# sunchao/leveldb-rs

Hardware: AMD Instinct MI355X
Metric: GiB/s device-resident batched CRC32C, 4KiB blocks; %HBM-peak at 1/2/4/8 GPUs (higher is better)
Workload: dtype u32

## Files before the change

leveldb-rs_amd/csrc/lvk/knobs.h:

```cpp
#pragma once

#if !defined(LVK_EXPERIMENT_BUILD) && ( \
    defined(LVK_STAGGER) || \
    defined(LVK_AL_ROWS) || \
    defined(LVK_MAX_PIECES) || \
    defined(LVK_WAL_TOUCH_HOPS) || \
    defined(LVK_SMALL_WAVES) || \
    defined(LVK_SEAL_FLUSH) || \
    defined(LVK_SST_ROWS) || \
    defined(LVK_SEAL_ROWS) || \
    defined(LVK_SST_RUN) || \
    defined(LVK_SORT_MIN_WGS) || \
    defined(LVK_SMALL_ROUNDS) || \
    defined(LVK_HASH_WGS_PER_CU) || \
    defined(LVK_PIPE_CHUNK_MB) || \
    defined(LVK_PIPE_FIRST_MB) || \
    defined(LVK_MEMCPY_THREADS) || \
    defined(LVK_PIPE_COPY_THREADS) || \
    defined(LVK_WAL_UNSORT) || \
    defined(LVK_MT_TILE) || \
    defined(LVK_MT_PREFIX) || \
    defined(LVK_SB_TILE) || \
    defined(LVK_SB_WAVE_COPY) || \
    defined(LVK_SB_COPY_LANES))
#error "LVK_* kernel switches select untested code paths; only experiment variants (LVK_EXPERIMENT_BUILD, tools/build_variant.sh) may set them"
#endif

#ifndef LVK_STAGGER
#define LVK_STAGGER 1u
#endif
#ifndef LVK_AL_ROWS
#define LVK_AL_ROWS 4
#endif
#ifndef LVK_MAX_PIECES
#define LVK_MAX_PIECES 4096
#endif
#ifndef LVK_WAL_TOUCH_HOPS
#define LVK_WAL_TOUCH_HOPS 16
#endif
#ifndef LVK_SMALL_WAVES
#define LVK_SMALL_WAVES 4
#endif
#ifndef LVK_SEAL_FLUSH
#define LVK_SEAL_FLUSH 16
#endif
#ifndef LVK_SST_ROWS
#define LVK_SST_ROWS 3
#endif
#ifndef LVK_SEAL_ROWS
#define LVK_SEAL_ROWS LVK_SST_ROWS
#endif
#ifndef LVK_SST_RUN
#define LVK_SST_RUN 4
#endif
#ifndef LVK_SORT_MIN_WGS
#define LVK_SORT_MIN_WGS 1024
#endif
#ifndef LVK_SMALL_ROUNDS
#define LVK_SMALL_ROUNDS 52
#endif
#ifndef LVK_PIPE_CHUNK_MB
#define LVK_PIPE_CHUNK_MB 32
#endif
#ifndef LVK_PIPE_FIRST_MB
#define LVK_PIPE_FIRST_MB 2
#endif
#ifndef LVK_MEMCPY_THREADS
#define LVK_MEMCPY_THREADS 8
#endif
#ifndef LVK_PIPE_COPY_THREADS
#define LVK_PIPE_COPY_THREADS 4
#endif
#ifndef LVK_HASH_WGS_PER_CU
#define LVK_HASH_WGS_PER_CU 8
#endif
#ifndef LVK_WAL_UNSORT
#define LVK_WAL_UNSORT 1
#endif
#ifndef LVK_MT_TILE
#define LVK_MT_TILE 512
#endif
#ifndef LVK_MT_PREFIX
#define LVK_MT_PREFIX 16
#endif
#ifndef LVK_SB_TILE
#define LVK_SB_TILE 1024
#endif
#ifndef LVK_SB_WAVE_COPY
#define LVK_SB_WAVE_COPY 64
#endif
#ifndef LVK_SB_COPY_LANES
#define LVK_SB_COPY_LANES 16
#endif
```

leveldb-rs_amd/csrc/wal_decode.hip:

```cpp
#include <hip/hip_runtime.h>

#include <algorithm>
#include <string>

#include "../../include/lvgpu/crc32c.h"
#include "../../include/lvgpu/wal.h"
#include "lv_internal.h"
#include "lvh.h"
#include "lvk/sort.h"

namespace lvk {

constexpr uint32_t kDecThreads = 256;
constexpr uint32_t kDecPer = 4;
constexpr uint32_t kDecTile = kDecThreads * kDecPer;
constexpr uint32_t kDecBlock = 32768;
constexpr uint32_t kDecHeader = 7;
constexpr uint32_t kDecMaxFrags = kDecBlock / kDecHeader + 1;
constexpr uint64_t kDecNone = ~0ull;

enum : uint32_t {
    kEvSkip = 0,
    kEvFull = 1,
    kEvFirst = 2,
    kEvMiddle = 3,
    kEvLast = 4,
    kEvType0 = 5,
    kEvUnknown = 6,
    kEvBadZero = 7,
    kEvBadLen = 8,
    kEvBadCrc = 9,
    kEvEof = 10,
    kEvStop = 11,
};

constexpr uint32_t kOpConst = 1, kOpIn = 2, kOpStop = 4;
struct DecOp {
    uint32_t flags;
    uint32_t pad;
    uint64_t size;
    uint64_t start;
};

__device__ __forceinline__ DecOp dec_ident() { return DecOp{0u, 0u, 0ull, 0ull}; }
__device__ __forceinline__ DecOp dec_closed() { return DecOp{kOpConst, 0u, 0ull, 0ull}; }

__device__ __forceinline__ DecOp dec_compose(const DecOp &a, const DecOp &b) {
    if (a.flags & kOpStop) return a;
    if (b.flags & kOpConst) return b;
    DecOp r = a;
    if (!(a.flags & kOpConst) || (a.flags & kOpIn)) r.size += b.size;
    return r;
}

__device__ __forceinline__ DecOp dec_event_op(uint32_t code, uint32_t x, uint64_t hdr) {
    if (code == kEvSkip) return dec_ident();
    if (code == kEvMiddle) return DecOp{0u, 0u, x, 0ull};
    if (code == kEvFirst) return DecOp{kOpConst | kOpIn, 0u, x, hdr};
    if (code == kEvStop) return DecOp{kOpConst | kOpStop, 0u, 0ull, 0ull};
    return dec_closed();
}

// ... 428 lines not shown
        for (uint32_t j = 0; j < kDecPer; ++j) {
            before[j] = (s.flags & kOpIn) ? s.size : kDecNone;
            if (s.flags & kOpStop) code[j] = kEvSkip;
            dec_step(code[j], x[j], hdr[j], &s, &v[j]);
            dec_accumulate(&sum, v[j]);
        }
        DecSum stotal;
        const DecSum ex = dec_scan_sum(sum, s_sum, &stotal);
        uint32_t all;
        uint32_t next = dec_next_nonzero(cfirst, s_code, &all);
        if (!next) next = ti.next_code;
        uint32_t nx[kDecPer];
#pragma unroll
        for (int j = kDecPer - 1; j >= 0; --j) {
            nx[j] = next;
            if (code[j] != kEvSkip && code[j] != kEvMiddle) next = code[j];
        }
        uint64_t R = ti.recs + ex.recs, P = ti.pay + ex.pay, Q = ti.reps + ex.reps;
#pragma unroll
        for (uint32_t j = 0; j < kDecPer; ++j) {
            const uint64_t i = tile * kDecTile + t * kDecPer + j;
            if (i >= n) break;
            for (uint32_t r = 0; r < v[j].nrep; ++r, ++Q) {
                if (!A.out.d_rep_bytes || Q >= A.out.rep_cap) continue;
                A.out.d_rep_bytes[Q] = v[j].rb[r];
                A.out.d_rep_reason[Q] = v[j].rr[r];
                A.out.d_rep_log_off[Q] = hdr[j];
            }
            uint64_t fp = kDecNone;
            if (code[j] == kEvFull)
                fp = P;
            else if (code[j] == kEvFirst && nx[j] == kEvLast)
                fp = P;
            else if (code[j] == kEvMiddle && before[j] != kDecNone && nx[j] == kEvLast)
                fp = P + before[j];
            else if (code[j] == kEvLast && before[j] != kDecNone)
                fp = P + before[j];
            A.fpos[i] = fp;
            if (v[j].emit) {
                if (R < A.out.rec_cap) {
                    A.out.d_rec_off[R] = P;
                    A.out.d_rec_len[R] = v[j].emit_len;
                    A.out.d_rec_log_off[R] = v[j].rec_log;
                }
                ++R;
                P += v[j].emit_len;
            }
        }
    }
}

typedef uint32_t dec_u4 __attribute__((ext_vector_type(4)));

__global__ __launch_bounds__(kDecThreads) void wal_unframe_kernel(const DecArgs A) {
    __shared__ uint16_t s_out[kDecMaxFrags + 1];
    __shared__ uint16_t s_src[kDecMaxFrags];
    __shared__ uint32_t s_wt[kDecThreads / 64];
    __shared__ uint64_t s_span;
    if (A.head->status) return;
    const uint32_t tid = threadIdx.x;
    const uint64_t n = A.head->n;
    const uint64_t nblocks = A.nblocks < A.nb ? A.nblocks : A.nb;
    for (uint64_t blk = blockIdx.x; blk < nblocks; blk += gridDim.x) {
        const uint32_t e0 = A.bfirst[blk], e1 = A.bend[blk];
        uint32_t cnt = 0;
        if (e0 != ~0u && e1 != ~0u && e1 > e0 && e1 <= n) cnt = e1 - e0 < kDecMaxFrags ? e1 - e0 : kDecMaxFrags;
        const uint64_t start = blk * kDecBlock;
        __syncthreads();
        uint32_t carry = 0;
        for (uint32_t k0 = 0; k0 < cnt; k0 += kDecThreads) {
            const uint32_t k = k0 + tid;
            uint32_t ll = 0;
            uint64_t fp = kDecNone;
            if (k < cnt) {
                const uint64_t i = static_cast<uint64_t>(e0) + k;
                fp = A.fpos[i];
                if (fp != kDecNone) ll = (A.ev[i] >> 8) & 0xffffu;
                s_src[k] = static_cast<uint16_t>(A.hdr_off[i] - start + kDecHeader);
            }
            const uint32_t inc = wg_incl_scan<kDecThreads / 64>(ll, s_wt);
            const uint32_t o = carry + inc - ll;
            if (k < cnt) {
                s_out[k] = static_cast<uint16_t>(o);
                if (fp != kDecNone && o == 0) s_span = fp;
            }
            uint32_t tot = 0;
#pragma unroll
            for (uint32_t w = 0; w < kDecThreads / 64; ++w) tot += s_wt[w];
            carry += tot;
            __syncthreads();
        }
        if (tid == 0) s_out[cnt] = static_cast<uint16_t>(carry);
        __syncthreads();
        const uint32_t total = carry;
        if (total == 0) continue;
        const uint64_t span = s_span;
        if (span > A.out.payload_cap || total > A.out.payload_cap - span) continue;
        uint8_t *const dst = A.out.d_payload + span;
        const uint8_t *const src = A.log + start;
        const uint32_t mis = static_cast<uint32_t>(reinterpret_cast<uintptr_t>(dst) & 15u);
        uint32_t head = (16u - mis) & 15u;
        if (head > total) head = total;
        const uint32_t ngran = (head ? 1u : 0u) + (total - head + 15u) / 16u;
        for (uint32_t g = tid; g < ngran; g += kDecThreads) {
            uint32_t lo, hi;
            if (head && g == 0) {
                lo = 0;
                hi = head;
            } else {
                lo = head + (g - (head ? 1u : 0u)) * 16u;
                hi = lo + 16u < total ? lo + 16u : total;
            }
            uint32_t a = 0, b = cnt;
            while (a < b) {
                const uint32_t m = (a + b) >> 1;
                if (s_out[m] <= lo)
                    a = m + 1;
                else
                    b = m;
            }
            uint32_t f = a - 1;
            if (hi - lo == 16u && lo + 16u <= s_out[f + 1]) {
                dec_u4 v;
                __builtin_memcpy(&v, src + s_src[f] + (lo - s_out[f]), 16);
                *reinterpret_cast<dec_u4 *>(dst + lo) = v;
                continue;
            }
            uint64_t wlo = 0, whi = 0;
            for (uint32_t p = lo; p < hi; ++p) {
                while (s_out[f + 1] <= p) ++f;
                const uint64_t byte = src[s_src[f] + (p - s_out[f])];
                const uint32_t q = p - lo;
                if (q < 8)
                    wlo |= byte << (8 * q);
                else
                    whi |= byte << (8 * (q - 8));
            }
            if (hi - lo == 16u) {
                dec_u4 v;
                v.x = static_cast<uint32_t>(wlo);
                v.y = static_cast<uint32_t>(wlo >> 32);
                v.z = static_cast<uint32_t>(whi);
                v.w = static_cast<uint32_t>(whi >> 32);
                *reinterpret_cast<dec_u4 *>(dst + lo) = v;
            } else {
                for (uint32_t q = 0; q < hi - lo; ++q)
                    dst[lo + q] = static_cast<uint8_t>((q < 8 ? wlo >> (8 * q) : whi >> (8 * (q - 8))) & 0xffu);
            }
        }
    }
}

}

using namespace lvh;

namespace {

constexpr uint64_t kMaxScanCap = 0xfffffffeull;

struct DecWs {
    size_t head, ev, fpos, blk, tsum, tin, total;
    uint64_t nb, tiles;
};
DecWs dec_ws_layout(uint64_t cap) {
    DecWs w;
    w.nb = cap + 1;
    w.tiles = (cap + lvk::kDecTile - 1) / lvk::kDecTile;
    w.head = 0;
    w.ev = al16(sizeof(lvk::DecHead));
    w.fpos = w.ev + al16(cap * sizeof(uint32_t));
    w.blk = w.fpos + al16(cap * sizeof(uint64_t));
    w.tsum = w.blk + al16(3 * w.nb * sizeof(uint32_t));
    w.tin = w.tsum + al16(w.tiles * sizeof(lvk::DecTileSum));
    w.total = w.tin + al16(w.tiles * sizeof(lvk::DecTileIn));
    return w;
}

}

extern "C" {

size_t lv_wal_decode_workspace_bytes(size_t scan_cap) { return dec_ws_layout(scan_cap).total; }

int lv_wal_decode_device(const uint8_t *d_log, size_t bytes, const uint64_t *d_hdr_off, const uint32_t *d_crc,
                         const uint32_t *d_info, const uint64_t *d_count, size_t scan_cap,
                         const lv_wal_decode_out *out, uint32_t flags, void *d_workspace, size_t workspace_bytes,
                         void *stream) {
    g_err.clear();
    if (flags & ~static_cast<uint32_t>(LV_WAL_DECODE_NO_CHECKSUM)) return set_err(LV_ERR_INVALID, "unknown flag bits");
    const bool checksum = !(flags & LV_WAL_DECODE_NO_CHECKSUM);
    if (!out) return set_err(LV_ERR_INVALID, "null output descriptor");
    if (!out->d_totals) return set_err(LV_ERR_INVALID, "null d_totals");
    if (reinterpret_cast<uintptr_t>(out->d_totals) % 8) return set_err(LV_ERR_INVALID, "d_totals must be 8-byte aligned");
    if (!d_count) return set_err(LV_ERR_INVALID, "null count pointer");
    if (!d_log && bytes) return set_err(LV_ERR_INVALID, "null log pointer");
    if (scan_cap && (!d_hdr_off || !d_info)) return set_err(LV_ERR_INVALID, "null scan array");
    if (scan_cap && checksum && !d_crc) return set_err(LV_ERR_INVALID, "null d_crc (only LV_WAL_DECODE_NO_CHECKSUM allows it)");
    if (out->payload_cap && !out->d_payload) return set_err(LV_ERR_INVALID, "null d_payload");
    if (out->rec_cap && (!out->d_rec_off || !out->d_rec_len || !out->d_rec_log_off))
// ... 65 lines not shown
```

leveldb-rs_amd/csrc/wal_encode.hip:

```cpp
#include <hip/hip_runtime.h>

#include <algorithm>
#include <cstring>
#include <mutex>
#include <vector>

#include "../../include/lvgpu/crc32c.h"
#include "../../include/lvgpu/wal.h"
#include "lv_internal.h"
#include "lvh.h"

namespace lvk {

constexpr uint32_t kFrameThreads = 256;
constexpr uint32_t kFrameBlock = 32768;
constexpr uint32_t kFrameHeader = 7;
constexpr uint32_t kFrameMaxFrags = kFrameBlock / kFrameHeader + 1;
constexpr uint64_t kFramePosMask = (1ull << 56) - 1;

struct FrameArgs {
    const uint8_t *payload;
    uint8_t *out;
    uint64_t out_len;
    uint32_t first;
    uint32_t align;
    uint64_t nblocks;
    uint64_t nfrags;
    const uint64_t *src;
    const uint64_t *pos;
    const uint32_t *len;
    const uint32_t *crc;
    const uint32_t *bidx;
};

typedef uint32_t frame_u4 __attribute__((ext_vector_type(4)));

struct FrameFrag {
    uint64_t pos, src, next;
    uint32_t len, crc, type;
};

__device__ __forceinline__ void frame_load(const FrameArgs &A, int64_t f, FrameFrag *r) {
    const uint64_t pw = A.pos[f];
    r->pos = pw & kFramePosMask;
    r->type = static_cast<uint32_t>(pw >> 56);
    r->src = A.src[f];
    r->len = A.len[f];
    r->crc = A.crc[f];
    r->next = static_cast<uint64_t>(f + 1) < A.nfrags ? (A.pos[f + 1] & kFramePosMask) : ~0ull;
}

__device__ __forceinline__ void frame_compose(const FrameArgs &A, int64_t p0, int64_t f) {
    FrameFrag r{};
    if (f >= 0)
        frame_load(A, f, &r);
    else
        r.next = A.nfrags ? (A.pos[0] & kFramePosMask) : ~0ull;
    uint64_t lo = 0, hi = 0;
    uint32_t valid = 0;
    for (uint32_t k = 0; k < 16; ++k) {
        const int64_t p = p0 + k;
        if (p < 0 || static_cast<uint64_t>(p) >= A.out_len) continue;
        valid |= 1u << k;
        while (static_cast<uint64_t>(p) >= r.next) frame_load(A, ++f, &r);
        uint32_t b = 0;
        if (f >= 0) {
            const uint64_t d = static_cast<uint64_t>(p) - r.pos;
            if (d < 4)
                b = (r.crc >> (8 * d)) & 0xffu;
            else if (d < 6)
                b = (r.len >> (8 * (d - 4))) & 0xffu;
            else if (d == 6)
                b = r.type;
            else if (d < kFrameHeader + r.len)
                b = A.payload[r.src + d - kFrameHeader];
        }
        if (k < 8)
            lo |= static_cast<uint64_t>(b) << (8 * k);
        else
            hi |= static_cast<uint64_t>(b) << (8 * (k - 8));
    }
    uint8_t *q = A.out + p0;
    if (valid == 0xffffu) {
        frame_u4 v;
        v.x = static_cast<uint32_t>(lo);
        v.y = static_cast<uint32_t>(lo >> 32);
        v.z = static_cast<uint32_t>(hi);
        v.w = static_cast<uint32_t>(hi >> 32);
        *reinterpret_cast<frame_u4 *>(q) = v;
    } else {
        for (uint32_t k = 0; k < 16; ++k)
            if (valid & (1u << k)) q[k] = static_cast<uint8_t>((k < 8 ? lo >> (8 * k) : hi >> (8 * (k - 8))) & 0xffu);
    }
}

__global__ __launch_bounds__(kFrameThreads) void wal_frame_kernel(const FrameArgs A) {
    __shared__ uint16_t s_pos[kFrameMaxFrags];
    const uint32_t tid = threadIdx.x;
    for (uint64_t blk = blockIdx.x; blk < A.nblocks; blk += gridDim.x) {
        const uint64_t lo = blk == 0 ? 0 : blk * kFrameBlock - A.first;
        const uint64_t end = (blk + 1) * kFrameBlock - A.first;
        const uint64_t hi = end < A.out_len ? end : A.out_len;
        const uint32_t f0 = A.bidx[blk];
        const uint32_t cnt = A.bidx[blk + 1] - f0;
        const uint32_t nf = cnt < kFrameMaxFrags ? cnt : kFrameMaxFrags;
        __syncthreads();
        for (uint32_t i = tid; i < nf; i += kFrameThreads)
            s_pos[i] = static_cast<uint16_t>((A.pos[f0 + i] & kFramePosMask) - lo);
        __syncthreads();
        const uint64_t g_lo = blk == 0 ? 0 : (lo + A.align + 15) / 16;
        const uint64_t g_hi = (hi + A.align + 15) / 16;
        for (uint64_t g = g_lo + tid; g < g_hi; g += kFrameThreads) {
            const int64_t p0 = static_cast<int64_t>(g * 16) - static_cast<int64_t>(A.align);
            const uint32_t rel = static_cast<uint32_t>((p0 < 0 ? 0 : p0) - static_cast<int64_t>(lo));
            uint32_t a = 0, b = nf;
            while (a < b) {
                const uint32_t m = (a + b) >> 1;
                if (s_pos[m] <= rel)
                    a = m + 1;
                else
                    b = m;
            }
            const int64_t f = static_cast<int64_t>(f0) + a - 1;
            if (a > 0 && p0 >= 0) {
                const uint32_t d = rel - s_pos[a - 1];
                const uint32_t len = A.len[f];
                if (d >= kFrameHeader && d + 16 <= kFrameHeader + len) {
                    frame_u4 v;
                    __builtin_memcpy(&v, A.payload + A.src[f] + (d - kFrameHeader), 16);
                    *reinterpret_cast<frame_u4 *>(A.out + p0) = v;
                    continue;
                }
            }
            frame_compose(A, p0, a > 0 ? f : static_cast<int64_t>(f0) - 1);
        }
    }
}

}

using namespace lvh;

namespace {

constexpr uint64_t kMaxFragments = 0xffffffffull;

struct EncWs {
    size_t src, pos, len, seed, bidx, crc, image, sort, total;
};
EncWs enc_ws_layout(uint64_t fragments) {
    EncWs w;
    w.src = 0;
    w.pos = w.src + al16(fragments * sizeof(uint64_t));
    w.len = w.pos + al16(fragments * sizeof(uint64_t));
    w.seed = w.len + al16(fragments * sizeof(uint32_t));
    w.bidx = w.seed + al16(fragments * sizeof(uint32_t));
    w.crc = w.bidx + al16((fragments + 2) * sizeof(uint32_t));
    w.image = w.crc + al16(fragments * sizeof(uint32_t));
    w.sort = w.image;
    w.total = w.sort + al16(lv_crc32c_workspace_bytes(fragments));
    return w;
}

struct StageSlot {
    uint8_t *p = nullptr;
    size_t cap = 0;
    int dev = -1;
    hipEvent_t done = nullptr;
    bool used = false;
    bool retired = false;
};
std::mutex g_stage_m;
std::vector<StageSlot> *g_stage = nullptr;

int stage_acquire(int dev, size_t need, size_t *slot) {
    if (!g_stage) g_stage = new std::vector<StageSlot>();
    std::vector<StageSlot> &v = *g_stage;
    for (size_t i = 0; i < v.size(); ++i) {
        if (v[i].dev != dev || v[i].cap < need || v[i].retired) continue;
        if (v[i].used && hipEventQuery(v[i].done) != hipSuccess) {
            (void)hipGetLastError();
            continue;
        }
        *slot = i;
        return LV_OK;
    }
    StageSlot s;
// ... 116 lines not shown
```

leveldb-rs_amd/csrc/sst_build.hip:

```cpp
#include <hip/hip_runtime.h>

#include <string>

#include "../../include/lvgpu/crc32c.h"
#include "../../include/lvgpu/table.h"
#include "lv_internal.h"
#include "lvh.h"
#include "lvk/knobs.h"

namespace lvk {

constexpr uint32_t kSbTile = LVK_SB_TILE;
constexpr uint32_t kSbWaveCopy = LVK_SB_WAVE_COPY;
constexpr uint32_t kSbCopyLanes = LVK_SB_COPY_LANES;
constexpr uint32_t kSbThreads = 256;
constexpr uint32_t kSbPer = kSbTile / kSbThreads;
constexpr uint32_t kSbMaxR = LV_SST_MAX_RESTART_INTERVAL;
constexpr uint64_t kSbLarge = 0xffffffffull;
static_assert(kSbTile % kSbThreads == 0 && kSbTile >= kSbMaxR, "a tile holds every residue of a restart interval");
static_assert(kSbTile * 16 <= 65536, "two u64 scan arrays fit the LDS a workgroup may declare");
static_assert(kSbWaveCopy >= 16, "a wave copy has at least one granule");
static_assert(kSbCopyLanes >= 16 && 64 % kSbCopyLanes == 0, "a copy's lanes cover a ragged head or tail of 15 bytes");

typedef uint32_t sb_u4 __attribute__((ext_vector_type(4)));
// ... 71 lines not shown
}

__device__ __forceinline__ void sb_put_fixed32(uint8_t *p, uint32_t v) {
    p[0] = static_cast<uint8_t>(v);
    p[1] = static_cast<uint8_t>(v >> 8);
    p[2] = static_cast<uint8_t>(v >> 16);
    p[3] = static_cast<uint8_t>(v >> 24);
}

__device__ __forceinline__ uint32_t sb_ikey_at(const uint8_t *k, uint64_t ulen, uint64_t tag, uint64_t i) {
    return i < ulen ? k[i] : static_cast<uint32_t>(tag >> (8 * (i - ulen))) & 0xffu;
}

__device__ __forceinline__ uint64_t sb_common(const uint8_t *a, const uint8_t *b, uint64_t m) {
    uint64_t i = 0;
    for (; i + 8 <= m; i += 8) {
        uint64_t x, y;
        __builtin_memcpy(&x, a + i, 8);
        __builtin_memcpy(&y, b + i, 8);
        if (x != y) return i + (static_cast<uint32_t>(__builtin_ctzll(x ^ y)) >> 3);
    }
    for (; i < m && a[i] == b[i]; ++i) {
    }
    return i;
}

__device__ __forceinline__ uint64_t sb_shared(const SbArgs &A, const lv_wb_op &p, const lv_wb_op &c) {
    const uint8_t *kp = A.payload + p.key_off, *kc = A.payload + c.key_off;
    const uint64_t m = p.key_len < c.key_len ? p.key_len : c.key_len;
    uint64_t s = sb_common(kp, kc, m);
    if (s < m) return s;
    for (uint32_t k = 0; k < 8; ++k, ++s)
        if (sb_ikey_at(kp, p.key_len, p.tag, s) != sb_ikey_at(kc, c.key_len, c.tag, s)) break;
    return s;
}

__device__ __forceinline__ void sb_tile_scan(uint64_t *s, uint32_t st, uint32_t tid) {
    for (uint32_t off = st; off < kSbTile; off <<= 1) {
        uint64_t v[kSbPer];
#pragma unroll
        for (uint32_t k = 0; k < kSbPer; ++k) {
            const uint32_t j = tid + k * kSbThreads;
            v[k] = j >= off ? s[j - off] : 0;
        }
        __syncthreads();
#pragma unroll
        for (uint32_t k = 0; k < kSbPer; ++k) s[tid + k * kSbThreads] += v[k];
        __syncthreads();
    }
}

__device__ __forceinline__ uint64_t sb_P(const SbArgs &A, uint64_t i) { return A.Pl[i] + A.cP[i / kSbTile]; }
__device__ __forceinline__ uint64_t sb_S(const SbArgs &A, uint64_t i) {
    return A.Sl[i] + A.cS[(i / kSbTile) * A.R + i % A.R];
}
__device__ __forceinline__ uint64_t sb_buffer(const SbArgs &A, uint64_t s, uint64_t e, uint64_t *restarts) {
    const uint64_t k = (e - s) / A.R, last = s + k * A.R;
    *restarts = k + 1;
    return sb_P(A, e) - (s ? sb_P(A, s - 1) : 0) + sb_S(A, last) - (s >= A.R ? sb_S(A, s - A.R) : 0);
}
__device__ __forceinline__ uint64_t sb_estimate(const SbArgs &A, uint64_t s, uint64_t e) {
    uint64_t r;
    const uint64_t b = sb_buffer(A, s, e, &r);
    return b + 4 * r + 4;
}

__global__ void sb_init(const SbArgs A) {
    SbHead h{};
    *A.head = h;
}

__global__ __launch_bounds__(kSbThreads) void sb_sizes(const SbArgs A) {
    __shared__ uint64_t s_p[kSbTile], s_s[kSbTile];
    const uint32_t tid = threadIdx.x;
    const uint64_t n = sb_entries(A);
    const uint64_t base = static_cast<uint64_t>(blockIdx.x) * kSbTile;
    if (base >= n) return;
    const uint32_t cnt = static_cast<uint32_t>(n - base < kSbTile ? n - base : kSbTile);
    int bad = 0;
#pragma unroll
    for (uint32_t k = 0; k < kSbPer; ++k) {
        const uint32_t j = tid + k * kSbThreads;
        uint64_t nr = 0, d = 0;
        if (j < cnt) {
            const uint64_t i = base + j;
            const uint32_t oi = A.order[i], pi = i ? A.order[i - 1] : oi;
            uint64_t sh = 0;
            if (oi >= A.op_cap || pi >= A.op_cap) {
                bad = 1;
            } else {
                const lv_wb_op o = sb_load_op(A.ops + oi), p = sb_load_op(A.ops + pi);
                if (!sb_extent_ok(o.key_off, o.key_len, A.payload_bytes) ||
                    !sb_extent_ok(o.val_off, o.val_len, A.payload_bytes) ||
                    !sb_extent_ok(p.key_off, p.key_len, A.payload_bytes)) {
                    bad = 1;
                } else {
                    if (i) sh = sb_shared(A, p, o);
                    const uint64_t klen = static_cast<uint64_t>(o.key_len) + 8, vlen = o.val_len;
                    nr = sb_varint_len(sh) + sb_varint_len(klen - sh) + sb_varint_len(vlen) + (klen - sh) + vlen;
                    d = 1 + sb_varint_len(klen) + sb_varint_len(vlen) + klen + vlen - nr;
                }
            }
            A.shared[i] = sh;
        }
        s_p[j] = nr;
        s_s[j] = d;
    }
    if (__syncthreads_or(bad)) {
        if (tid == 0) atomicOr(&A.head->bad, 1u);
        return;
// ... 179 lines not shown
            if (b < A.block_cap) {
                A.blk_start[b] = static_cast<uint32_t>(s);
                A.wsh[2 * b] = off;
                A.wsh[2 * b + 1] = raw;
            }
            v = sb_index_entry(A, e, n, sb_load_op(A.ops + A.order[e]), off, raw).size;
        }
        s_i[j] = v;
    }
    __syncthreads();
    sb_tile_scan(s_i, 1, tid);
#pragma unroll
    for (uint32_t k = 0; k < kSbPer; ++k) {
        const uint32_t j = tid + k * kSbThreads;
        if (j < cnt) A.Il[base + j] = s_i[j];
    }
    if (tid == 0) A.cI[blockIdx.x] = s_i[cnt - 1];
}

__global__ void sb_plan(const SbArgs A) {
    SbHead *h = A.head;
    lv_sst_build_totals t{};
    uint64_t n = A.mt->entries;
    if (A.mt->status || n > A.op_cap || h->bad) {
        t.status = LV_SST_BUILD_NO_TABLE;
        n = 0;
    }
    t.entries = n;
    if (n) {
        const uint64_t nb = h->nblocks;
        t.data_blocks = nb;
        t.metaindex_offset = h->data_bytes;
        t.metaindex_size = 8;
        t.index_offset = t.metaindex_offset + 8 + LV_SST_TRAILER_SIZE;
        t.index_size = h->idx_bytes + 4 * nb + 4;
        t.file_bytes = t.index_offset + t.index_size + LV_SST_TRAILER_SIZE + LV_SST_FOOTER_SIZE;
        if (h->large || t.index_size >= kSbLarge) t.status |= LV_SST_BUILD_BLOCK_LARGE;
        if (nb > A.block_cap) t.status |= LV_SST_BUILD_HANDLE_OVER;
        if (t.file_bytes > A.file_cap) t.status |= LV_SST_BUILD_FILE_OVER;
        if (!t.status) {
            h->go = 1;
            h->meta_off = t.metaindex_offset;
            h->index_off = t.index_offset;
            h->index_size = t.index_size;
            A.wsh[2 * nb] = t.metaindex_offset;
            A.wsh[2 * nb + 1] = t.metaindex_size;
            A.wsh[2 * nb + 2] = t.index_offset;
            A.wsh[2 * nb + 3] = t.index_size;
        }
    }
    *A.totals = t;
}

__device__ __forceinline__ void sb_wave_copy(uint8_t *dst, const uint8_t *src, uint64_t len, uint32_t lane) {
    const uint32_t head = static_cast<uint32_t>((16u - (reinterpret_cast<uintptr_t>(dst) & 15u)) & 15u);
    const uint64_t gran = (len - head) / 16;
    const uint32_t tail = static_cast<uint32_t>((len - head) % 16);
    if (lane < head) dst[lane] = src[lane];
    for (uint64_t g = lane; g < gran; g += kSbCopyLanes) {
        sb_u4 v;
        __builtin_memcpy(&v, src + head + g * 16, 16);
        *reinterpret_cast<sb_u4 *>(dst + head + g * 16) = v;
    }
    if (lane < tail) dst[head + gran * 16 + lane] = src[head + gran * 16 + lane];
}

__device__ __forceinline__ void sb_copy(uint8_t *dst, const uint8_t *src, uint64_t len, uint32_t lane) {
    constexpr uint32_t kGroups = 64 / kSbCopyLanes;
    if (len < kSbWaveCopy)
        for (uint64_t i = 0; i < len; ++i) dst[i] = src[i];
    uint64_t todo = __ballot(len >= kSbWaveCopy);
    const uint32_t grp = lane / kSbCopyLanes;
    while (todo) {
        int l = -1;
        uint64_t t = todo;
#pragma unroll
        for (uint32_t k = 0; k < kGroups; ++k) {
            if (k <= grp) l = t ? __ffsll(static_cast<unsigned long long>(t)) - 1 : -1;
            t &= t - 1;
        }
        todo = t;
        const int from = l < 0 ? 0 : l;
        uint8_t *d = reinterpret_cast<uint8_t *>(__shfl(reinterpret_cast<unsigned long long>(dst), from, 64));
        const uint8_t *sp = reinterpret_cast<const uint8_t *>(__shfl(reinterpret_cast<unsigned long long>(src), from, 64));
        const uint64_t m = __shfl(static_cast<unsigned long long>(len), from, 64);
        if (l >= 0) sb_wave_copy(d, sp, m, lane % kSbCopyLanes);
    }
}

__global__ __launch_bounds__(kSbThreads) void sb_emit(const SbArgs A) {
    if (!A.head->go) return;
    const uint32_t lane = threadIdx.x & 63u;
    const uint64_t n = sb_entries(A);
    const uint64_t i = static_cast<uint64_t>(blockIdx.x) * kSbThreads + threadIdx.x;
    if (static_cast<uint64_t>(blockIdx.x) * kSbThreads >= n) return;
    const bool on = i < n;
    uint8_t *kd = nullptr, *vd = nullptr, *xd = nullptr;
    const uint8_t *ks = nullptr, *vs = nullptr, *xs = nullptr;
    uint64_t kn = 0, vn = 0, xn = 0;
    if (on) {
        const lv_wb_op o = sb_load_op(A.ops + A.order[i]);
        const uint64_t b = A.Cl[i] + A.cC[i / kSbTile] - 1;
        const uint64_t s = A.blk_start[b], boff = A.wsh[2 * b], raw = A.wsh[2 * b + 1];
        const bool restart = (i - s) % A.R == 0;
        uint64_t r;
        const uint64_t rel = i > s ? sb_buffer(A, s, i - 1, &r) : 0;
        const uint64_t ulen = o.key_len, klen = ulen + 8, sh = restart ? 0 : A.shared[i];
        uint8_t *p = A.file + boff + rel;
        p = sb_put_varint(p, sh);
        p = sb_put_varint(p, klen - sh);
        p = sb_put_varint(p, o.val_len);
        if (sh < ulen) {
            kd = p;
            ks = A.payload + o.key_off + sh;
            kn = ulen - sh;
            p += kn;
        }
        for (uint32_t t = sh > ulen ? static_cast<uint32_t>(sh - ulen) : 0; t < 8; ++t)
            *p++ = static_cast<uint8_t>(o.tag >> (8 * t));
        vd = p;
        vs = A.payload + o.val_off;
        vn = o.val_len;
        const uint64_t cnt = static_cast<uint64_t>(A.nxt[s]) - s, nrest = (cnt + A.R - 1) / A.R;
        uint8_t *arr = A.file + boff + raw - 4 - 4 * nrest;
        if (restart) sb_put_fixed32(arr + 4 * ((i - s) / A.R), static_cast<uint32_t>(rel));
        if (i == s) {
            sb_put_fixed32(arr + 4 * nrest, static_cast<uint32_t>(nrest));
            const uint64_t e = s + cnt - 1;
            const lv_wb_op le = sb_load_op(A.ops + A.order[e]);
            const SbIndexEntry x = sb_index_entry(A, e, n, le, boff, raw);
            const uint64_t at = A.Il[i] + A.cI[i / kSbTile] - x.size;
            uint8_t *ix = A.file + A.head->index_off;
            sb_put_fixed32(ix + A.head->idx_bytes + 4 * b, static_cast<uint32_t>(at));
            uint8_t *q = ix + at;
            q = sb_put_varint(q, 0);
            q = sb_put_varint(q, x.klen);
            q = sb_put_varint(q, x.hlen);
            xd = q;
            xs = A.payload + le.key_off;
            xn = x.sep.copy;
            q += xn;
            uint64_t tg = le.tag;
            if (x.sep.bump) {
                *q++ = static_cast<uint8_t>(xs[xn] + 1);
                tg = (LV_MT_MAX_SEQUENCE << 8) | 1u;
            }
            for (uint32_t t = 0; t < 8; ++t) *q++ = static_cast<uint8_t>(tg >> (8 * t));
            q = sb_put_varint(q, boff);
            q = sb_put_varint(q, raw);
        }
    }
    sb_copy(kd, ks, kn, lane);
    sb_copy(vd, vs, vn, lane);
    if (__ballot(xn != 0)) sb_copy(xd, xs, xn, lane);
}

__global__ __launch_bounds__(kSbThreads) void sb_tail(const SbArgs A) {
    const SbHead *h = A.head;
    const uint64_t j = static_cast<uint64_t>(blockIdx.x) * kSbThreads + threadIdx.x;
    const bool go = h->go;
    const uint64_t nh = go ? h->nblocks + 2 : 0;
    if (j < A.block_cap + 2) {
        if (j < nh) {
            A.handles[2 * j] = A.wsh[2 * j];
            A.handles[2 * j + 1] = A.wsh[2 * j + 1];
        }
        if (j + 1 >= nh) {
            A.wsh[2 * j] = ~0ull;
            A.wsh[2 * j + 1] = 0;
        }
    }
    if (j == 0) {
        A.idx_off[0] = go ? h->index_off : 0;
        A.idx_len[0] = go ? static_cast<uint32_t>(h->index_size + 1) : 0;
    }
    if (j == 0 && go) {
        A.file[h->index_off + h->index_size] = LV_SST_NO_COMPRESSION;
        uint8_t *m = A.file + h->meta_off;
        sb_put_fixed32(m, 0);
        sb_put_fixed32(m + 4, 1);
        sb_put_fixed32(A.file + h->index_off + h->idx_bytes + 4 * h->nblocks, static_cast<uint32_t>(h->nblocks));
        uint8_t *f = A.file + h->index_off + h->index_size + LV_SST_TRAILER_SIZE, *q = f;
        q = sb_put_varint(q, h->meta_off);
        q = sb_put_varint(q, 8);
        q = sb_put_varint(q, h->index_off);
        q = sb_put_varint(q, h->index_size);
        while (q < f + 40) *q++ = 0;
        for (uint32_t t = 0; t < 8; ++t) *q++ = static_cast<uint8_t>(LV_SST_MAGIC >> (8 * t));
    }
}

__global__ void sb_index_trailer(const SbArgs A) {
    const SbHead *h = A.head;
    if (h->go) sb_put_fixed32(A.file + h->index_off + h->index_size + 1, A.idx_crc[0]);
}

}

using namespace lvh;

namespace {

constexpr uint64_t kMaxOpCap = 0xfffffffeull;
constexpr uint64_t kMaxBlockCap = 0xfffffffcull;

struct SbWs {
    size_t head, shared, Pl, Sl, cP, cS, nxt, J0, J1, F, Cl, Bl, Il, cC, cB, cI, blk_start, wsh, idx, crc_ws, crc_ws_bytes, total;
// ... 173 lines not shown
```

Before: 6079.

## Batch WAL frame/unframe copies into per-lane strips with staged fragment metadata

Restructures the WAL frame and unframe copy loops so each lane handles K granules at once. It runs an interleaved branchless binary search over all K, issues all K 16-byte loads, waits once, then does the stores, with the rare boundary granules handled afterwards. The frame kernel also stages per-fragment src and len in LDS, and the unframe kernel prefetches the next block's entry bounds. The aim is more memory-level parallelism and fewer global metadata reads, at the cost of more registers and LDS and some risk of lower occupancy. This targets the WAL kernels rather than the CRC32C metric being measured.

```diff
diff --git a/leveldb-rs_amd/csrc/lvk/knobs.h b/leveldb-rs_amd/csrc/lvk/knobs.h
--- a/leveldb-rs_amd/csrc/lvk/knobs.h
+++ b/leveldb-rs_amd/csrc/lvk/knobs.h
@@ -22,7 +22,10 @@
     defined(LVK_MT_PREFIX) || \
     defined(LVK_SB_TILE) || \
     defined(LVK_SB_WAVE_COPY) || \
-    defined(LVK_SB_COPY_LANES))
+    defined(LVK_SB_COPY_LANES) || \
+    defined(LVK_WAL_STAGE_FRAGS) || \
+    defined(LVK_WAL_STRIP) || \
+    defined(LVK_WAL_UNFRAME_STRIP))
 #error "LVK_* kernel switches select untested code paths; only experiment variants (LVK_EXPERIMENT_BUILD, tools/build_variant.sh) may set them"
 #endif
 
@@ -92,3 +95,12 @@
 #ifndef LVK_SB_COPY_LANES
 #define LVK_SB_COPY_LANES 16
 #endif
+#ifndef LVK_WAL_STAGE_FRAGS
+#define LVK_WAL_STAGE_FRAGS 1024
+#endif
+#ifndef LVK_WAL_STRIP
+#define LVK_WAL_STRIP 4
+#endif
+#ifndef LVK_WAL_UNFRAME_STRIP
+#define LVK_WAL_UNFRAME_STRIP 8
+#endif
diff --git a/leveldb-rs_amd/csrc/lvk/strips.h b/leveldb-rs_amd/csrc/lvk/strips.h
--- /dev/null
+++ b/leveldb-rs_amd/csrc/lvk/strips.h
@@ -0,0 +1,50 @@
+#pragma once
+
+#include <stdint.h>
+
+namespace lvk {
+
+struct StripGranule {
+    uint32_t g;
+    bool has;
+};
+template <uint32_t T>
+__device__ __forceinline__ StripGranule strip_granule(uint32_t s, uint32_t k, uint32_t t, uint32_t n) {
+    const uint32_t g = (s + k) * T + t;
+    return StripGranule{g < n ? g : n - 1u, g < n};
+}
+
+template <uint32_t K>
+__device__ __forceinline__ void strip_search(const uint16_t *tab, uint32_t n, const uint32_t (&key)[K],
+                                             uint32_t (&idx)[K]) {
+#pragma unroll
+    for (uint32_t k = 0; k < K; ++k) idx[k] = 0;
+    if (n == 0) return;
+    uint32_t left = n;
+    while (left > 1) {
+        const uint32_t half = left >> 1;
+#pragma unroll
+        for (uint32_t k = 0; k < K; ++k)
+            if (tab[idx[k] + half - 1] <= key[k]) idx[k] += half;
+        left -= half;
+    }
+#pragma unroll
+    for (uint32_t k = 0; k < K; ++k)
+        if (tab[idx[k]] <= key[k]) ++idx[k];
+}
+
+typedef uint32_t strip_u4 __attribute__((ext_vector_type(4)));
+typedef strip_u4 strip_u4_unaligned __attribute__((aligned(1)));
+
+__device__ __forceinline__ strip_u4 strip_load16(const uint8_t *p) {
+    return *reinterpret_cast<const __attribute__((address_space(1))) strip_u4_unaligned *>(
+        reinterpret_cast<uintptr_t>(p));
+}
+
+__device__ __forceinline__ void strip_wait_vm() { __builtin_amdgcn_s_waitcnt((7 << 4) | (15 << 8)); }
+
+__device__ __forceinline__ void strip_store16(uint8_t *p, strip_u4 v) {
+    *reinterpret_cast<__attribute__((address_space(1))) strip_u4 *>(reinterpret_cast<uintptr_t>(p)) = v;
+}
+
+}
diff --git a/leveldb-rs_amd/csrc/wal_decode.hip b/leveldb-rs_amd/csrc/wal_decode.hip
--- a/leveldb-rs_amd/csrc/wal_decode.hip
+++ b/leveldb-rs_amd/csrc/wal_decode.hip
@@ -7,7 +7,9 @@
 #include "../../include/lvgpu/wal.h"
 #include "lv_internal.h"
 #include "lvh.h"
+#include "lvk/knobs.h"
 #include "lvk/sort.h"
+#include "lvk/strips.h"
 
 namespace lvk {
 
@@ -542,21 +544,60 @@
 
 typedef uint32_t dec_u4 __attribute__((ext_vector_type(4)));
 
+__device__ __forceinline__ void unframe_compose(const uint16_t *s_out, const uint16_t *s_src, const uint8_t *src,
+                                                uint8_t *dst, uint32_t lo, uint32_t hi, uint32_t f) {
+    uint64_t wlo = 0, whi = 0;
+    for (uint32_t p = lo; p < hi; ++p) {
+        while (s_out[f + 1] <= p) ++f;
+        const uint64_t byte = src[s_src[f] + (p - s_out[f])];
+        const uint32_t q = p - lo;
+        if (q < 8)
+            wlo |= byte << (8 * q);
+        else
+            whi |= byte << (8 * (q - 8));
+    }
+    if (hi - lo == 16u) {
+        dec_u4 v;
+        v.x = static_cast<uint32_t>(wlo);
+        v.y = static_cast<uint32_t>(wlo >> 32);
+        v.z = static_cast<uint32_t>(whi);
+        v.w = static_cast<uint32_t>(whi >> 32);
+        *reinterpret_cast<dec_u4 *>(dst + lo) = v;
+    } else {
+        for (uint32_t q = 0; q < hi - lo; ++q)
+            dst[lo + q] = static_cast<uint8_t>((q < 8 ? wlo >> (8 * q) : whi >> (8 * (q - 8))) & 0xffu);
+    }
+}
+
+__device__ __forceinline__ uint32_t unframe_lo(uint32_t g, uint32_t head) {
+    return head && g == 0 ? 0u : head + (g - (head ? 1u : 0u)) * 16u;
+}
+
 __global__ __launch_bounds__(kDecThreads) void wal_unframe_kernel(const DecArgs A) {
     __shared__ uint16_t s_out[kDecMaxFrags + 1];
     __shared__ uint16_t s_src[kDecMaxFrags];
     __shared__ uint32_t s_wt[kDecThreads / 64];
+    __shared__ uint32_t s_ent[2];
     __shared__ uint64_t s_span;
+    constexpr uint32_t K = LVK_WAL_UNFRAME_STRIP;
+    static_assert(K == 4 || K == 8, "LVK_WAL_UNFRAME_STRIP: 4 or 8 granules per lane");
     if (A.head->status) return;
     const uint32_t tid = threadIdx.x;
     const uint64_t n = A.head->n;
     const uint64_t nblocks = A.nblocks < A.nb ? A.nblocks : A.nb;
+    const uint8_t *__restrict__ const log = A.log;
+    uint8_t *__restrict__ const payload = A.out.d_payload;
+    const uint32_t *const ent = tid == 0 ? A.bfirst : A.bend;
+    uint32_t nv = ~0u;
+    if (tid < 2 && blockIdx.x < nblocks) nv = ent[blockIdx.x];
     for (uint64_t blk = blockIdx.x; blk < nblocks; blk += gridDim.x) {
-        const uint32_t e0 = A.bfirst[blk], e1 = A.bend[blk];
+        if (tid < 2) s_ent[tid] = nv;
+        __syncthreads();
+        const uint32_t e0 = s_ent[0], e1 = s_ent[1];
+        if (tid < 2 && blk + gridDim.x < nblocks) nv = ent[blk + gridDim.x];
         uint32_t cnt = 0;
         if (e0 != ~0u && e1 != ~0u && e1 > e0 && e1 <= n) cnt = e1 - e0 < kDecMaxFrags ? e1 - e0 : kDecMaxFrags;
         const uint64_t start = blk * kDecBlock;
-        __syncthreads();
         uint32_t carry = 0;
         for (uint32_t k0 = 0; k0 < cnt; k0 += kDecThreads) {
             const uint32_t k = k0 + tid;
@@ -586,56 +627,45 @@
         if (total == 0) continue;
         const uint64_t span = s_span;
         if (span > A.out.payload_cap || total > A.out.payload_cap - span) continue;
-        uint8_t *const dst = A.out.d_payload + span;
-        const uint8_t *const src = A.log + start;
+        uint8_t *const dst = payload + span;
+        const uint8_t *const src = log + start;
         const uint32_t mis = static_cast<uint32_t>(reinterpret_cast<uintptr_t>(dst) & 15u);
         uint32_t head = (16u - mis) & 15u;
         if (head > total) head = total;
         const uint32_t ngran = (head ? 1u : 0u) + (total - head + 15u) / 16u;
-        for (uint32_t g = tid; g < ngran; g += kDecThreads) {
-            uint32_t lo, hi;
-            if (head && g == 0) {
-                lo = 0;
-                hi = head;
-            } else {
-                lo = head + (g - (head ? 1u : 0u)) * 16u;
-                hi = lo + 16u < total ? lo + 16u : total;
-            }
-            uint32_t a = 0, b = cnt;
-            while (a < b) {
-                const uint32_t m = (a + b) >> 1;
-                if (s_out[m] <= lo)
-                    a = m + 1;
-                else
-                    b = m;
-            }
-            uint32_t f = a - 1;
-            if (hi - lo == 16u && lo + 16u <= s_out[f + 1]) {
-                dec_u4 v;
-                __builtin_memcpy(&v, src + s_src[f] + (lo - s_out[f]), 16);
-                *reinterpret_cast<dec_u4 *>(dst + lo) = v;
-                continue;
-            }
-            uint64_t wlo = 0, whi = 0;
-            for (uint32_t p = lo; p < hi; ++p) {
-                while (s_out[f + 1] <= p) ++f;
-                const uint64_t byte = src[s_src[f] + (p - s_out[f])];
-                const uint32_t q = p - lo;
-                if (q < 8)
-                    wlo |= byte << (8 * q);
-                else
-                    whi |= byte << (8 * (q - 8));
-            }
-            if (hi - lo == 16u) {
-                dec_u4 v;
-                v.x = static_cast<uint32_t>(wlo);
-                v.y = static_cast<uint32_t>(wlo >> 32);
-                v.z = static_cast<uint32_t>(whi);
-                v.w = static_cast<uint32_t>(whi >> 32);
-                *reinterpret_cast<dec_u4 *>(dst + lo) = v;
-            } else {
-                for (uint32_t q = 0; q < hi - lo; ++q)
-                    dst[lo + q] = static_cast<uint8_t>((q < 8 ? wlo >> (8 * q) : whi >> (8 * (q - 8))) & 0xffu);
+        for (uint32_t st = 0; st * kDecThreads < ngran; st += K) {
+            uint32_t lo[K], a[K];
+            uint32_t rest = 0;
+            bool whole[K];
+            uint32_t from[K];
+#pragma unroll
+            for (uint32_t k = 0; k < K; ++k) lo[k] = unframe_lo(strip_granule<kDecThreads>(st, k, tid, ngran).g, head);
+            strip_search<K>(s_out, cnt, lo, a);
+#pragma unroll
+            for (uint32_t k = 0; k < K; ++k) {
+                const StripGranule sg = strip_granule<kDecThreads>(st, k, tid, ngran);
+                const uint32_t f = a[k] - 1;
+                whole[k] = sg.has && !(head && sg.g == 0) && lo[k] + 16u <= s_out[f + 1];
+                from[k] = s_src[f] + (lo[k] - s_out[f]);
+                if (sg.has && !whole[k]) rest |= 1u << k;
+            }
+            strip_u4 v[K];
+#pragma unroll
+            for (uint32_t k = 0; k < K; ++k)
+                if (whole[k]) v[k] = strip_load16(src + from[k]);
+            strip_wait_vm();
+#pragma unroll
+            for (uint32_t k = 0; k < K; ++k)
+                if (whole[k]) strip_store16(dst + lo[k], v[k]);
+            while (rest) {
+                const uint32_t k = static_cast<uint32_t>(__builtin_ctz(rest));
+                rest &= rest - 1u;
+                const uint32_t g = (st + k) * kDecThreads + tid;
+                const uint32_t l[1] = {unframe_lo(g, head)};
+                uint32_t c[1];
+                strip_search<1>(s_out, cnt, l, c);
+                const uint32_t h = head && g == 0 ? head : (l[0] + 16u < total ? l[0] + 16u : total);
+                unframe_compose(s_out, s_src, src, dst, l[0], h, c[0] - 1);
             }
         }
     }
diff --git a/leveldb-rs_amd/csrc/wal_encode.hip b/leveldb-rs_amd/csrc/wal_encode.hip
--- a/leveldb-rs_amd/csrc/wal_encode.hip
+++ b/leveldb-rs_amd/csrc/wal_encode.hip
@@ -9,6 +9,8 @@
 #include "../../include/lvgpu/wal.h"
 #include "lv_internal.h"
 #include "lvh.h"
+#include "lvk/knobs.h"
+#include "lvk/strips.h"
 
 namespace lvk {
 
@@ -17,6 +19,8 @@
 constexpr uint32_t kFrameHeader = 7;
 constexpr uint32_t kFrameMaxFrags = kFrameBlock / kFrameHeader + 1;
 constexpr uint64_t kFramePosMask = (1ull << 56) - 1;
+constexpr uint32_t kFrameStage = LVK_WAL_STAGE_FRAGS;
+static_assert(LVK_WAL_STRIP == 4 || LVK_WAL_STRIP == 8, "LVK_WAL_STRIP: 4 or 8 granules per lane");
 
 struct FrameArgs {
     const uint8_t *payload;
@@ -94,9 +98,24 @@
     }
 }
 
+struct FrameLds {
+    uint64_t src[kFrameStage];
+    uint16_t pos[kFrameMaxFrags];
+    uint16_t len[kFrameStage];
+};
+static_assert(sizeof(FrameLds) <= 20480, "wal_frame_kernel: 8 workgroups per CU share 160 KiB of LDS");
+
+__device__ __forceinline__ uint32_t frame_rel(int32_t rel0, uint32_t g) {
+    const int32_t r = rel0 + static_cast<int32_t>(g * 16u);
+    return static_cast<uint32_t>(r < 0 ? 0 : r);
+}
+
 __global__ __launch_bounds__(kFrameThreads) void wal_frame_kernel(const FrameArgs A) {
-    __shared__ uint16_t s_pos[kFrameMaxFrags];
+    __shared__ FrameLds s;
+    constexpr uint32_t K = LVK_WAL_STRIP;
     const uint32_t tid = threadIdx.x;
+    const uint8_t *__restrict__ const payload = A.payload;
+    uint8_t *__restrict__ const out = A.out;
     for (uint64_t blk = blockIdx.x; blk < A.nblocks; blk += gridDim.x) {
         const uint64_t lo = blk == 0 ? 0 : blk * kFrameBlock - A.first;
         const uint64_t end = (blk + 1) * kFrameBlock - A.first;
@@ -104,35 +123,75 @@
         const uint32_t f0 = A.bidx[blk];
         const uint32_t cnt = A.bidx[blk + 1] - f0;
         const uint32_t nf = cnt < kFrameMaxFrags ? cnt : kFrameMaxFrags;
+        const uint32_t ns = nf < kFrameStage ? nf : kFrameStage;
         __syncthreads();
-        for (uint32_t i = tid; i < nf; i += kFrameThreads)
-            s_pos[i] = static_cast<uint16_t>((A.pos[f0 + i] & kFramePosMask) - lo);
+        for (uint32_t i = tid; i < ns; i += kFrameThreads) {
+            const uint64_t pw = A.pos[f0 + i], src = A.src[f0 + i];
+            const uint32_t len = A.len[f0 + i];
+            s.pos[i] = static_cast<uint16_t>((pw & kFramePosMask) - lo);
+            s.len[i] = static_cast<uint16_t>(len);
+            s.src[i] = src;
+        }
+        for (uint32_t i = ns + tid; i < nf; i += kFrameThreads)
+            s.pos[i] = static_cast<uint16_t>((A.pos[f0 + i] & kFramePosMask) - lo);
         __syncthreads();
         const uint64_t g_lo = blk == 0 ? 0 : (lo + A.align + 15) / 16;
         const uint64_t g_hi = (hi + A.align + 15) / 16;
-        for (uint64_t g = g_lo + tid; g < g_hi; g += kFrameThreads) {
-            const int64_t p0 = static_cast<int64_t>(g * 16) - static_cast<int64_t>(A.align);
-            const uint32_t rel = static_cast<uint32_t>((p0 < 0 ? 0 : p0) - static_cast<int64_t>(lo));
-            uint32_t a = 0, b = nf;
-            while (a < b) {
-                const uint32_t m = (a + b) >> 1;
-                if (s_pos[m] <= rel)
-                    a = m + 1;
-                else
-                    b = m;
+        const uint32_t ngran = static_cast<uint32_t>(g_hi - g_lo);
+        const int32_t rel0 = static_cast<int32_t>(static_cast<int64_t>(g_lo * 16) - static_cast<int64_t>(A.align) -
+                                                  static_cast<int64_t>(lo));
+        for (uint32_t st = 0; st * kFrameThreads < ngran; st += K) {
+            uint32_t rel[K], a[K];
+            uint32_t rest = 0;
+            bool interior[K];
+            const uint8_t *from[K];
+#pragma unroll
+            for (uint32_t k = 0; k < K; ++k)
+                rel[k] = frame_rel(rel0, strip_granule<kFrameThreads>(st, k, tid, ngran).g);
+            strip_search<K>(s.pos, nf, rel, a);
+#pragma unroll
+            for (uint32_t k = 0; k < K; ++k) {
+                const bool has = strip_granule<kFrameThreads>(st, k, tid, ngran).has;
+                interior[k] = false;
+                from[k] = payload;
+                if (has && a[k] > 0) {
+                    const uint32_t i = a[k] - 1;
+                    const uint32_t d = rel[k] - s.pos[i];
+                    uint32_t len;
+                    uint64_t src;
+                    if (i < ns) {
+                        len = s.len[i];
+                        src = s.src[i];
+                    } else {
+                        len = A.len[f0 + i];
+                        src = A.src[f0 + i];
+                        strip_wait_vm();
+                    }
+                    if (d >= kFrameHeader && d + 16 <= kFrameHeader + len) {
+                        interior[k] = true;
+                        from[k] = payload + src + (d - kFrameHeader);
+                    }
+                }
+                if (has && !interior[k]) rest |= 1u << k;
             }
-            const int64_t f = static_cast<int64_t>(f0) + a - 1;
-            if (a > 0 && p0 >= 0) {
-                const uint32_t d = rel - s_pos[a - 1];
-                const uint32_t len = A.len[f];
-                if (d >= kFrameHeader && d + 16 <= kFrameHeader + len) {
-                    frame_u4 v;
-                    __builtin_memcpy(&v, A.payload + A.src[f] + (d - kFrameHeader), 16);
-                    *reinterpret_cast<frame_u4 *>(A.out + p0) = v;
-                    continue;
-                }
+            strip_u4 v[K];
+#pragma unroll
+            for (uint32_t k = 0; k < K; ++k)
+                if (interior[k]) v[k] = strip_load16(from[k]);
+            strip_wait_vm();
+#pragma unroll
+            for (uint32_t k = 0; k < K; ++k)
+                if (interior[k]) strip_store16(out + lo + rel[k], v[k]);
+            while (rest) {
+                const uint32_t k = static_cast<uint32_t>(__builtin_ctz(rest));
+                rest &= rest - 1u;
+                const uint32_t g = (st + k) * kFrameThreads + tid;
+                const uint32_t r[1] = {frame_rel(rel0, g)};
+                uint32_t c[1];
+                strip_search<1>(s.pos, nf, r, c);
+                const int64_t p0 = rel0 < 0 && g == 0 ? static_cast<int64_t>(rel0) : static_cast<int64_t>(lo + r[0]);
+                frame_compose(A, p0, static_cast<int64_t>(f0) + c[0] - 1);
             }
-            frame_compose(A, p0, a > 0 ? f : static_cast<int64_t>(f0) - 1);
         }
     }
 }
```

Measured after the change: 6079 (median of 3 runs). Within noise of the previous version (+0.0%).

## Speed up SST emit copies with overlapping lane copies, unrolled wave copies, 32-bit divides

Applied to the files above, without the earlier changes.

Replaces the per-byte loop for short key/value copies with overlapping 16/8/4-byte vector copies, and unrolls the wave-cooperative copy four granules deep so each lane has several loads in flight. Head and tail bytes are loaded before the main loop. Destinations are carried as offsets into the file buffer so alignment comes from the offset. Restart and division arithmetic is narrowed to 32-bit, and fixed32 writes use aligned stores when possible. This trims per-entry instruction count and memory latency in the emit kernel, at the cost of redundant overlapping writes and an assumption that intra-block indices fit in 32 bits.

```diff
diff --git a/leveldb-rs_amd/csrc/sst_build.hip b/leveldb-rs_amd/csrc/sst_build.hip
--- a/leveldb-rs_amd/csrc/sst_build.hip
+++ b/leveldb-rs_amd/csrc/sst_build.hip
@@ -147,10 +147,10 @@
 
 __device__ __forceinline__ uint64_t sb_P(const SbArgs &A, uint64_t i) { return A.Pl[i] + A.cP[i / kSbTile]; }
 __device__ __forceinline__ uint64_t sb_S(const SbArgs &A, uint64_t i) {
-    return A.Sl[i] + A.cS[(i / kSbTile) * A.R + i % A.R];
+    return A.Sl[i] + A.cS[(i / kSbTile) * A.R + static_cast<uint32_t>(i) % A.R];
 }
 __device__ __forceinline__ uint64_t sb_buffer(const SbArgs &A, uint64_t s, uint64_t e, uint64_t *restarts) {
-    const uint64_t k = (e - s) / A.R, last = s + k * A.R;
+    const uint64_t k = static_cast<uint32_t>(e - s) / A.R, last = s + k * A.R;
     *restarts = k + 1;
     return sb_P(A, e) - (s ? sb_P(A, s - 1) : 0) + sb_S(A, last) - (s >= A.R ? sb_S(A, s - A.R) : 0);
 }
@@ -436,23 +436,76 @@
     *A.totals = t;
 }
 
-__device__ __forceinline__ void sb_wave_copy(uint8_t *dst, const uint8_t *src, uint64_t len, uint32_t lane) {
-    const uint32_t head = static_cast<uint32_t>((16u - (reinterpret_cast<uintptr_t>(dst) & 15u)) & 15u);
+__device__ __forceinline__ void sb_put_fixed32_at(uint8_t *base, uint64_t off, uint32_t v) {
+    if (off % 4 == 0)
+        *reinterpret_cast<uint32_t *>(base + off) = v;
+    else
+        sb_put_fixed32(base + off, v);
+}
+
+__device__ __forceinline__ void sb_lane_copy(uint8_t *w, const uint8_t *src, uint32_t n) {
+    if (n >= 16) {
+        const uint32_t m = n - 16;
+        for (uint32_t i = 0; i < n; i += 64) {
+            const uint32_t a0 = i < m ? i : m, a1 = i + 16 < m ? i + 16 : m, a2 = i + 32 < m ? i + 32 : m,
+                           a3 = i + 48 < m ? i + 48 : m;
+            sb_u4 v0, v1, v2, v3;
+            __builtin_memcpy(&v0, src + a0, 16);
+            __builtin_memcpy(&v1, src + a1, 16);
+            __builtin_memcpy(&v2, src + a2, 16);
+            __builtin_memcpy(&v3, src + a3, 16);
+            __builtin_memcpy(w + a0, &v0, 16);
+            __builtin_memcpy(w + a1, &v1, 16);
+            __builtin_memcpy(w + a2, &v2, 16);
+            __builtin_memcpy(w + a3, &v3, 16);
+        }
+    } else if (n >= 8) {
+        uint64_t a, b;
+        __builtin_memcpy(&a, src, 8);
+        __builtin_memcpy(&b, src + n - 8, 8);
+        __builtin_memcpy(w, &a, 8);
+        __builtin_memcpy(w + n - 8, &b, 8);
+    } else if (n >= 4) {
+        uint32_t a, b;
+        __builtin_memcpy(&a, src, 4);
+        __builtin_memcpy(&b, src + n - 4, 4);
+        __builtin_memcpy(w, &a, 4);
+        __builtin_memcpy(w + n - 4, &b, 4);
+    } else if (n) {
+        const uint8_t a = src[0], b = src[n / 2], c = src[n - 1];
+        w[0] = a;
+        w[n / 2] = b;
+        w[n - 1] = c;
+    }
+}
+
+__device__ __forceinline__ void sb_wave_copy(uint8_t *dst, uint32_t mis, const uint8_t *src, uint64_t len, uint32_t lane) {
+    const uint32_t head = (16u - mis) & 15u;
     const uint64_t gran = (len - head) / 16;
     const uint32_t tail = static_cast<uint32_t>((len - head) % 16);
-    if (lane < head) dst[lane] = src[lane];
-    for (uint64_t g = lane; g < gran; g += kSbCopyLanes) {
-        sb_u4 v;
-        __builtin_memcpy(&v, src + head + g * 16, 16);
-        *reinterpret_cast<sb_u4 *>(dst + head + g * 16) = v;
-    }
-    if (lane < tail) dst[head + gran * 16 + lane] = src[head + gran * 16 + lane];
-}
-
-__device__ __forceinline__ void sb_copy(uint8_t *dst, const uint8_t *src, uint64_t len, uint32_t lane) {
+    const uint64_t e0 = lane < head ? lane : 0, e1 = lane < tail ? head + gran * 16 + lane : 0;
+    const uint8_t hb = src[e0], tb = src[e1];
+    for (uint64_t g = lane; g < gran; g += 4 * kSbCopyLanes) {
+        constexpr uint32_t L = kSbCopyLanes;
+        const uint64_t a0 = head + g * 16, a1 = head + (g + L < gran ? g + L : g) * 16;
+        const uint64_t a2 = head + (g + 2 * L < gran ? g + 2 * L : g) * 16, a3 = head + (g + 3 * L < gran ? g + 3 * L : g) * 16;
+        sb_u4 v0, v1, v2, v3;
+        __builtin_memcpy(&v0, src + a0, 16);
+        __builtin_memcpy(&v1, src + a1, 16);
+        __builtin_memcpy(&v2, src + a2, 16);
+        __builtin_memcpy(&v3, src + a3, 16);
+        *reinterpret_cast<sb_u4 *>(dst + a0) = v0;
+        *reinterpret_cast<sb_u4 *>(dst + a1) = v1;
+        *reinterpret_cast<sb_u4 *>(dst + a2) = v2;
+        *reinterpret_cast<sb_u4 *>(dst + a3) = v3;
+    }
+    if (lane < head) dst[e0] = hb;
+    if (lane < tail) dst[e1] = tb;
+}
+
+__device__ __forceinline__ void sb_copy(uint8_t *file, uint64_t doff, const uint8_t *src, uint64_t len, uint32_t lane) {
     constexpr uint32_t kGroups = 64 / kSbCopyLanes;
-    if (len < kSbWaveCopy)
-        for (uint64_t i = 0; i < len; ++i) dst[i] = src[i];
+    if (len < kSbWaveCopy) sb_lane_copy(file + doff, src, static_cast<uint32_t>(len));
     uint64_t todo = __ballot(len >= kSbWaveCopy);
     const uint32_t grp = lane / kSbCopyLanes;
     while (todo) {
@@ -465,10 +518,10 @@
         }
         todo = t;
         const int from = l < 0 ? 0 : l;
-        uint8_t *d = reinterpret_cast<uint8_t *>(__shfl(reinterpret_cast<unsigned long long>(dst), from, 64));
+        const uint64_t d = __shfl(static_cast<unsigned long long>(doff), from, 64);
         const uint8_t *sp = reinterpret_cast<const uint8_t *>(__shfl(reinterpret_cast<unsigned long long>(src), from, 64));
         const uint64_t m = __shfl(static_cast<unsigned long long>(len), from, 64);
-        if (l >= 0) sb_wave_copy(d, sp, m, lane % kSbCopyLanes);
+        if (l >= 0) sb_wave_copy(file + d, static_cast<uint32_t>(d) & 15u, sp, m, lane % kSbCopyLanes);
     }
 }
 
@@ -479,14 +532,15 @@
     const uint64_t i = static_cast<uint64_t>(blockIdx.x) * kSbThreads + threadIdx.x;
     if (static_cast<uint64_t>(blockIdx.x) * kSbThreads >= n) return;
     const bool on = i < n;
-    uint8_t *kd = nullptr, *vd = nullptr, *xd = nullptr;
+    uint64_t kd = 0, vd = 0, xd = 0;
     const uint8_t *ks = nullptr, *vs = nullptr, *xs = nullptr;
     uint64_t kn = 0, vn = 0, xn = 0;
     if (on) {
         const lv_wb_op o = sb_load_op(A.ops + A.order[i]);
         const uint64_t b = A.Cl[i] + A.cC[i / kSbTile] - 1;
         const uint64_t s = A.blk_start[b], boff = A.wsh[2 * b], raw = A.wsh[2 * b + 1];
-        const bool restart = (i - s) % A.R == 0;
+        const uint32_t run = static_cast<uint32_t>(i - s) / A.R;
+        const bool restart = static_cast<uint32_t>(i - s) == run * A.R;
         uint64_t r;
         const uint64_t rel = i > s ? sb_buffer(A, s, i - 1, &r) : 0;
         const uint64_t ulen = o.key_len, klen = ulen + 8, sh = restart ? 0 : A.shared[i];
@@ -495,38 +549,39 @@
         p = sb_put_varint(p, klen - sh);
         p = sb_put_varint(p, o.val_len);
         if (sh < ulen) {
-            kd = p;
+            kd = static_cast<uint64_t>(p - A.file);
             ks = A.payload + o.key_off + sh;
             kn = ulen - sh;
             p += kn;
         }
         for (uint32_t t = sh > ulen ? static_cast<uint32_t>(sh - ulen) : 0; t < 8; ++t)
             *p++ = static_cast<uint8_t>(o.tag >> (8 * t));
-        vd = p;
+        vd = static_cast<uint64_t>(p - A.file);
         vs = A.payload + o.val_off;
         vn = o.val_len;
-        const uint64_t cnt = static_cast<uint64_t>(A.nxt[s]) - s, nrest = (cnt + A.R - 1) / A.R;
-        uint8_t *arr = A.file + boff + raw - 4 - 4 * nrest;
-        if (restart) sb_put_fixed32(arr + 4 * ((i - s) / A.R), static_cast<uint32_t>(rel));
+        const uint64_t cnt = static_cast<uint64_t>(A.nxt[s]) - s, nrest = static_cast<uint32_t>(cnt - 1) / A.R + 1;
+        const uint64_t arr = boff + raw - 4 - 4 * nrest;
+        if (restart) sb_put_fixed32_at(A.file, arr + 4 * run, static_cast<uint32_t>(rel));
         if (i == s) {
-            sb_put_fixed32(arr + 4 * nrest, static_cast<uint32_t>(nrest));
+            sb_put_fixed32_at(A.file, arr + 4 * nrest, static_cast<uint32_t>(nrest));
             const uint64_t e = s + cnt - 1;
             const lv_wb_op le = sb_load_op(A.ops + A.order[e]);
             const SbIndexEntry x = sb_index_entry(A, e, n, le, boff, raw);
             const uint64_t at = A.Il[i] + A.cI[i / kSbTile] - x.size;
-            uint8_t *ix = A.file + A.head->index_off;
-            sb_put_fixed32(ix + A.head->idx_bytes + 4 * b, static_cast<uint32_t>(at));
-            uint8_t *q = ix + at;
+            const uint64_t io = A.head->index_off;
+            xs = A.payload + le.key_off;
+            xn = x.sep.copy;
+            const uint8_t up = x.sep.bump ? xs[xn] : 0;
+            sb_put_fixed32_at(A.file, io + A.head->idx_bytes + 4 * b, static_cast<uint32_t>(at));
+            uint8_t *q = A.file + io + at;
             q = sb_put_varint(q, 0);
             q = sb_put_varint(q, x.klen);
             q = sb_put_varint(q, x.hlen);
-            xd = q;
-            xs = A.payload + le.key_off;
-            xn = x.sep.copy;
+            xd = static_cast<uint64_t>(q - A.file);
             q += xn;
             uint64_t tg = le.tag;
             if (x.sep.bump) {
-                *q++ = static_cast<uint8_t>(xs[xn] + 1);
+                *q++ = static_cast<uint8_t>(up + 1);
                 tg = (LV_MT_MAX_SEQUENCE << 8) | 1u;
             }
             for (uint32_t t = 0; t < 8; ++t) *q++ = static_cast<uint8_t>(tg >> (8 * t));
@@ -534,9 +589,9 @@
             q = sb_put_varint(q, raw);
         }
     }
-    sb_copy(kd, ks, kn, lane);
-    sb_copy(vd, vs, vn, lane);
-    if (__ballot(xn != 0)) sb_copy(xd, xs, xn, lane);
+    sb_copy(A.file, kd, ks, kn, lane);
+    sb_copy(A.file, vd, vs, vn, lane);
+    if (__ballot(xn != 0)) sb_copy(A.file, xd, xs, xn, lane);
 }
 
 __global__ __launch_bounds__(kSbThreads) void sb_tail(const SbArgs A) {
```

Result: no change. 6026 before, 6024 after (-0.0%).
